# yanglei18/SGV3D

Measured on AMD Instinct MI355X. Metric: camera frames/sec at 864x1536->BEV, higher is better.
Workload: dtype f32

## Files before the change

include/sgv3d_hip.h:

```cpp
#ifndef SGV3D_HIP_H
#define SGV3D_HIP_H

#include <stddef.h>
#include <stdint.h>

#ifdef __cplusplus
extern "C" {
#endif

#define SGV3D_OK 0
#define SGV3D_EINVAL (-1)
#define SGV3D_ELAUNCH (-2)
#define SGV3D_ENOSPACE (-3)

const char *sgv3d_last_error(void);
int sgv3d_abi_version(void);


int sgv3d_voxel_pooling_forward(int batch_size, int num_points, int num_channels,
                                int num_voxel_x, int num_voxel_y, int num_voxel_z,
                                const int32_t *geom_xyz, const float *input_features,
                                float *output_features, int32_t *pos_memo, void *stream);
int sgv3d_voxel_pooling_forward_fresh(int batch_size, int num_points, int num_channels,
                                      int num_voxel_x, int num_voxel_y, int num_voxel_z,
// ... 193 lines not shown

int sgv3d_dense(int batch, int k, int n, const float *x, const float *w, const float *scale,
                const float *bias, int act, float *y, void *stream);
int sgv3d_dense_gated(int batch, int k, int n, const float *x, const float *w, const float *scale,
                      const float *bias, int act, float *y, const int32_t *run, void *stream);

int sgv3d_broadcast_channels(int batch, int pixels, int channels, int y_ld, int y_coff,
                             const float *v, float *y, void *stream);

int sgv3d_scale_channels(int batch, int pixels, int channels, const float *x, const float *gate,
                         float *y, void *stream);

int sgv3d_copy_channels(int batch, int pixels, int channels, int x_ld, int x_coff, const float *x,
                        float *y, void *stream);

int sgv3d_upsample_bilinear2x(int batch, int h, int w, int channels, const float *x, float *y, void *stream);

int sgv3d_add_mul_sigmoid(long long n, const float *a, const float *b, const float *c, float *y, void *stream);

int sgv3d_bsm_compose(int batch, int pixels, int num_depth, int context_channels, int semantic_channels,
                      int ld, const float *semantic_logits, int semantic_ld, float background_threshold,
                      float *height_context, void *stream);

int sgv3d_deform_conv3x3_forward(int batch, int h, int w, int channels, int groups, int out_per_group, const float *x,
                                 const float *offset, int off_ld, const float *const *w_packed, int k_pad, int cout_pad,
                                 float *y, int y_ld, int y_coff, void *stream);

size_t sgv3d_deform_conv3x3_bf16_weight_bytes(int channels, int groups, int out_per_group);
int sgv3d_deform_conv3x3_bf16_pack_weight(const float *weight, int channels, int groups, int out_per_group, void *w_packed,
                                          void *stream);
int sgv3d_deform_conv3x3_forward_bf16(int batch, int h, int w, int channels, int groups, int out_per_group, const void *x,
                                      int x_is_bf16, const float *offset, int off_ld, const void *w_packed, void *y,
                                      int y_is_bf16, int y_ld, int y_coff, void *stream);

int sgv3d_deform_im2col3x3(int batch, int h, int w, int channels, int groups, const float *x,
                           const float *offset, int off_ld, float *col, void *stream);

int sgv3d_head_final_conv(int batch, int h, int w, int num_branches, int hidden_ch, int total_out,
                          const float *hidden, const float *weight, const float *bias,
                          const int32_t *branch_of_out, float *out, void *stream);

size_t sgv3d_centerhead_branches_workspace_bytes(int batch, int h, int w, int total_out);
int sgv3d_centerhead_branches_forward(int batch, int h, int w, int cin, int x_ld, int x_coff, const float *x,
                                      int num_branches, const float *w1_wino, const float *scale1,
                                      const float *bias1, int total_out, const float *w2, const float *bias2,
                                      const int32_t *out_begin, float *out, void *workspace,
                                      size_t workspace_bytes, void *stream);

size_t sgv3d_centerhead_f4_weight_floats(int num_branches);
int sgv3d_centerhead_f4_pack_weight(const float *w1, int num_branches, float *u_packed, void *stream);
int sgv3d_centerhead_branches_forward_f4(int batch, int h, int w, int cin, int x_ld, int x_coff, const float *x,
                                         int num_branches, const float *u_packed, const float *scale1,
                                         const float *bias1, int total_out, const float *w2, const float *bias2,
                                         const int32_t *out_begin, float *out, void *workspace,
                                         size_t workspace_bytes, void *stream);

size_t sgv3d_conv3x3_f4res_weight_floats(int cout, int cin);
int sgv3d_conv3x3_f4res_pack_weight(const float *w, int cout, int cin_real, int cin, float *u_packed, void *stream);
int sgv3d_conv3x3_f4res_forward(const sgv3d_conv_desc *d, const float *x, const float *u_packed, const float *scale,
                                const float *bias, const float *residual, float *y, void *stream);

size_t sgv3d_centerhead_bf16_weight_bytes(int num_branches);
int sgv3d_centerhead_bf16_pack_weight(const float *w1, int num_branches, int cin, void *w1_packed, void *stream);
size_t sgv3d_centerhead_bf16_weight2_bytes(int num_branches);
int sgv3d_centerhead_bf16_pack_weight2(const float *w2, const int32_t *out_begin, int num_branches, void *w2_packed,
                                       void *stream);
// ... 451 lines not shown
```

sgv3d_amd/_lib.py:

```python
import ctypes
import os

_HERE = os.path.dirname(os.path.abspath(__file__))
LIB_PATH = os.path.join(_HERE, "csrc", "libsgv3d_hip.so")

c_int, c_void_p, c_size_t, c_ll = ctypes.c_int, ctypes.c_void_p, ctypes.c_size_t, ctypes.c_longlong


class ConvDesc(ctypes.Structure):
    _fields_ = [(n, c_int) for n in (
        "batch", "in_h", "in_w", "cin", "out_h", "out_w", "cout", "kh", "kw", "stride", "pad", "dil",
        "x_ld", "x_coff", "y_ld", "y_coff", "res_ld", "relu", "mode", "deconv_ks", "k_pad", "cout_pad",
        "tile", "x_nchw", "k_order", "split_k")]


class VitAttnDesc(ctypes.Structure):
    _fields_ = [(n, c_int) for n in ("batch", "height", "width", "heads", "head_dim", "win_h", "win_w")]


CONV_NORMAL, CONV_DECONV, CONV_NCHW_OUT, CONV_GROUP_PLANES = 0, 1, 2, 3
TILE_AUTO, TILE_128x128, TILE_128x64, TILE_64x128, TILE_64x64 = 0, 1, 2, 3, 4

_PROTOS = {
    "sgv3d_last_error": (ctypes.c_char_p, []),
# ... 69 lines not shown
    "sgv3d_conv_dw_bf16_forward_splitk": (c_int, [ctypes.POINTER(ConvDesc)] + [c_void_p] * 7 + [c_size_t, c_void_p]),
    "sgv3d_conv_dw_bf16_pair_forward": (c_int, [ctypes.POINTER(ConvDesc)] + [c_void_p] * 4 + [c_int] + [c_void_p] * 4 + [c_int, c_void_p, c_int, c_int, c_int, c_void_p]),
    "sgv3d_conv_winograd_weight_floats": (c_size_t, [c_int, c_int]),
    "sgv3d_conv_winograd_pack_weight": (c_int, [c_void_p, c_int, c_int, c_int, c_void_p, c_void_p]),
    "sgv3d_conv2d_winograd_forward": (c_int, [ctypes.POINTER(ConvDesc)] + [c_void_p] * 8 + [c_size_t, c_void_p]),
    "sgv3d_conv_winograd4_pack_weight": (c_int, [c_void_p, c_int, c_int, c_int, c_int, c_void_p, c_void_p]),
    "sgv3d_conv_winograd4_pack_weight_x3": (c_int, [c_void_p, c_int, c_int, c_int, c_int, c_void_p, c_void_p]),
    "sgv3d_conv_pack_weight_x3": (c_int, [c_void_p, c_int, c_int, c_int, c_int, c_int, c_int, c_void_p, c_void_p]),
    "sgv3d_conv2d_x3_forward": (c_int, [c_void_p] * 8 + [c_size_t, c_void_p]),
    "sgv3d_conv2d_x3_shortcut_forward": (c_int, [c_void_p] * 12),
    "sgv3d_stem_pool_x3_forward": (c_int, [c_int] * 3 + [c_void_p, c_void_p, c_size_t] + [c_void_p] * 3 + [c_int, c_int, c_void_p]),
    "sgv3d_conv2d_winograd4_workspace_bytes": (c_size_t, [ctypes.POINTER(ConvDesc)]),
    "sgv3d_conv2d_winograd4_forward": (c_int, [ctypes.POINTER(ConvDesc)] + [c_void_p] * 7 + [c_size_t, c_void_p]),
    "sgv3d_maxpool3x3s2": (c_int, [c_int] * 4 + [c_void_p] * 3),
    "sgv3d_maxpool3x3s2_bf16": (c_int, [c_int] * 4 + [c_void_p] * 3),
    "sgv3d_nchw_to_nhwc": (c_int, [c_int] * 5 + [c_void_p] * 3),
    "sgv3d_nhwc_to_nchw": (c_int, [c_int] * 6 + [c_void_p] * 3),
    "sgv3d_global_avgpool_workspace_bytes": (c_size_t, [c_int] * 2),
    "sgv3d_global_avgpool": (c_int, [c_int] * 4 + [c_void_p] * 3 + [c_size_t, c_void_p]),
    "sgv3d_dense": (c_int, [c_int] * 3 + [c_void_p] * 4 + [c_int, c_void_p, c_void_p]),
    "sgv3d_broadcast_channels": (c_int, [c_int] * 5 + [c_void_p] * 3),
    "sgv3d_scale_channels": (c_int, [c_int] * 3 + [c_void_p] * 4),
    "sgv3d_copy_channels": (c_int, [c_int] * 5 + [c_void_p] * 3),
    "sgv3d_upsample_bilinear2x": (c_int, [c_int] * 4 + [c_void_p] * 3),
    "sgv3d_add_mul_sigmoid": (c_int, [c_ll] + [c_void_p] * 5),
    "sgv3d_bsm_compose": (c_int, [c_int] * 6 + [c_void_p, c_int, ctypes.c_float, c_void_p, c_void_p]),
    "sgv3d_deform_im2col3x3": (c_int, [c_int] * 5 + [c_void_p, c_void_p, c_int, c_void_p, c_void_p]),
    "sgv3d_deform_conv3x3_forward": (c_int, [c_int] * 6 + [c_void_p, c_void_p, c_int, c_void_p, c_int, c_int, c_void_p, c_int, c_int,
                                                          c_void_p]),
    "sgv3d_deform_conv3x3_bf16_weight_bytes": (c_size_t, [c_int] * 3),
    "sgv3d_deform_conv3x3_bf16_pack_weight": (c_int, [c_void_p, c_int, c_int, c_int, c_void_p, c_void_p]),
    "sgv3d_deform_conv3x3_forward_bf16": (c_int, [c_int] * 6 + [c_void_p, c_int, c_void_p, c_int, c_void_p, c_void_p, c_int, c_int, c_int,
                                                               c_void_p]),
    "sgv3d_head_final_conv": (c_int, [c_int] * 6 + [c_void_p] * 6),
    "sgv3d_centerpoint_decode_workspace_bytes": (c_size_t, [c_int] * 3),
    "sgv3d_centerpoint_decode": (c_int, [c_int] * 5 + [c_void_p] * 6 + [c_ll] + [ctypes.c_float] * 6 +
                                 [ctypes.POINTER(ctypes.c_float), c_int, ctypes.c_float, c_int, c_void_p, c_size_t] +
                                 [c_void_p] * 6),
    "sgv3d_centerpoint_decode_tasks_workspace_bytes": (c_size_t, [c_int] * 4),
    "sgv3d_centerpoint_decode_tasks": (c_int, [c_int, c_int, ctypes.POINTER(ctypes.c_int32), c_int, c_int, c_int] +
                                       [ctypes.POINTER(c_void_p)] * 6 + [c_ll] + [ctypes.c_float] * 6 +
                                       [ctypes.POINTER(ctypes.c_float), c_int, ctypes.POINTER(ctypes.c_float), c_int, c_void_p,
                                        c_size_t] + [c_void_p] * 6),
    "sgv3d_centerpoint_merge_tasks": (c_int, [c_int] * 3 + [c_void_p] * 4 + [ctypes.POINTER(ctypes.c_int32)] + [c_void_p] * 5),
    "sgv3d_rotated_bev_iou_host": (c_int, [c_int] + [ctypes.POINTER(ctypes.c_float)] * 3),
    "sgv3d_rotate_nms_workspace_bytes": (c_size_t, [c_int] * 3),
    "sgv3d_rotate_nms": (c_int, [c_int] * 3 + [c_void_p] * 3 + [ctypes.c_float, ctypes.POINTER(ctypes.c_float), c_int, c_int,
                                                                ctypes.POINTER(ctypes.c_float), c_void_p, c_size_t, c_void_p, c_void_p]),
    "sgv3d_centerpoint_decode_tasks_rotate_workspace_bytes": (c_size_t, [c_int] * 4),
    "sgv3d_centerpoint_decode_tasks_rotate": (c_int, [c_int, c_int, ctypes.POINTER(ctypes.c_int32), c_int, c_int, c_int] +
                                              [ctypes.POINTER(c_void_p)] * 6 + [c_ll] + [ctypes.c_float] * 6 +
                                              [ctypes.POINTER(ctypes.c_float), c_int, ctypes.c_float, ctypes.POINTER(ctypes.c_float),
                                               c_int, c_int, ctypes.POINTER(ctypes.c_float), c_void_p, c_size_t] + [c_void_p] * 6),
    "sgv3d_centerhead_targets": (c_int, [c_int, c_int, c_void_p, c_void_p, c_int, ctypes.POINTER(ctypes.c_int32)] +
                                 [c_int] * 3 + [ctypes.c_float] * 5 + [ctypes.c_double, c_int, c_int] + [c_void_p] * 5),
    "sgv3d_conv2d_backward_weight_workspace_bytes": (c_size_t, [ctypes.POINTER(ConvDesc), c_int]),
    "sgv3d_conv2d_backward_weight": (c_int, [ctypes.POINTER(ConvDesc)] + [c_void_p] * 3 + [c_int, c_void_p, c_size_t, c_void_p]),
    "sgv3d_conv2d_backward_weight_bf16_workspace_bytes": (c_size_t, [ctypes.POINTER(ConvDesc), c_int]),
    "sgv3d_conv2d_backward_weight_bf16": (c_int, [ctypes.POINTER(ConvDesc)] + [c_void_p] * 3 + [c_int, c_void_p, c_size_t, c_void_p]),
    "sgv3d_conv2d_backward_weight_bf16_batched_workspace_bytes": (c_size_t, [ctypes.POINTER(ConvDesc), c_int, c_int]),
    "sgv3d_conv2d_backward_weight_bf16_batched": (c_int, [ctypes.POINTER(ConvDesc), c_void_p, ctypes.POINTER(c_void_p), ctypes.POINTER(c_void_p), c_int, c_int, c_void_p, c_size_t, c_void_p]),
    "sgv3d_conv2d_backward_weight_bf16_alltaps_workspace_bytes": (c_size_t, [ctypes.POINTER(ConvDesc), c_int, c_int]),
    "sgv3d_conv2d_backward_weight_bf16_alltaps": (c_int, [ctypes.POINTER(ConvDesc)] + [c_void_p] * 3 + [c_int, c_void_p, c_size_t, c_void_p]),
    "sgv3d_conv2d_backward_weight_bf16_tensors_workspace_bytes": (c_size_t, [ctypes.POINTER(ConvDesc), c_int]),
    "sgv3d_conv2d_backward_weight_bf16_tensors": (c_int, [ctypes.POINTER(ConvDesc)] + [c_void_p] * 3 + [c_int, c_void_p, c_size_t, c_void_p]),
    "sgv3d_conv2d_backward_weight_bf16_alltaps_tensors_workspace_bytes": (c_size_t, [ctypes.POINTER(ConvDesc), c_int]),
# ... 139 lines not shown
```

sgv3d_amd/csrc/dcn_fused_bf16.hip:

```cpp
#include "conv_common.hpp"

using namespace sgv3d;

namespace {

typedef float f32x4 __attribute__((ext_vector_type(4)));
typedef __bf16 bf16x8 __attribute__((ext_vector_type(8)));
typedef __bf16 bf16x4 __attribute__((ext_vector_type(4)));
typedef unsigned u32x4 __attribute__((ext_vector_type(4)));

constexpr int BK = 32;
constexpr int BM = 64;
constexpr int BN = 128;
constexpr int kThreads = 256;
constexpr int kMaxGroups = 8;
constexpr int kFragB = 64 * 16;
constexpr unsigned kOutside = 0x80000000u;

struct DcnBfArgs {
    const void *x;
    const float *off;
    const void *w;
    void *y;
    int H, W, C, cpg, opg, groups;
    int M;
    int off_ld, y_ld, y_coff;
    int nkt;
    int nchunk;
    int tiles_m;
    unsigned x_bytes, w_bytes;
};

__global__ __launch_bounds__(64) void dcn_bf16_pack_kernel(const float *__restrict__ w, int cpg, int opg, int nkt, int nblk,
                                                           __bf16 *__restrict__ out) {
    const int id = blockIdx.x;
    const int kt = id % nkt, gnb = id / nkt;
    const int nb = gnb % nblk, g = gnb / nblk;
    const int kpt = cpg / BK;
    const int tap = kt / kpt, cb = kt - tap * kpt;
    const int l = threadIdx.x;
    const int co = nb * 16 + (l & 15);
    __bf16 *dst = out + ((size_t)id * 64 + l) * 8;
#pragma unroll
    for (int j = 0; j < 8; ++j) {
        const int ci = cb * BK + 8 * (l >> 4) + j;
        dst[j] = co < opg ? (__bf16)w[((size_t)(g * opg + co) * cpg + ci) * 9 + tap] : (__bf16)0.f;
    }
}

__device__ __forceinline__ float as_f32(unsigned u) { return __builtin_bit_cast(float, u); }
// ... 42 lines not shown
        pw = (int)((unsigned)mm - t2 * a.W);
        const unsigned b = t2 / (unsigned)a.H;
        ph = (int)(t2 - b * a.H);
        pbase = (unsigned)(((size_t)b * a.H * a.W * a.C + (size_t)grp * a.cpg + c * 8) * ESZ);
    }
    char *const st_ptr = smem + r * (BK * 2) + ((c ^ ((r >> 2) & 3)) * 16);

    const int wave = tid >> 6, lane = tid & 63;
    const int l16 = lane & 15, lq = lane >> 4;
    const int rd_off = l16 * (BK * 2) + ((lq ^ ((l16 >> 2) & 3)) * 16);
    const int col0 = chunk * BN + 32 * wave;
    const bool live0 = col0 < a.opg, live1 = col0 + 16 < a.opg;
    const int nblk = 8 * a.nchunk;
    const int nb0 = grp * nblk + chunk * 8 + 2 * wave;
    const unsigned w_off0 = (unsigned)((size_t)nb0 * a.nkt * kFragB + lane * 16);
    const unsigned w_off1 = w_off0 + (unsigned)(a.nkt * kFragB);

    f32x4 acc[2][4];
#pragma unroll
    for (int nb = 0; nb < 2; ++nb)
#pragma unroll
        for (int mb = 0; mb < 4; ++mb) acc[nb][mb] = f32x4{0.f, 0.f, 0.f, 0.f};

    unsigned co[4];
    float cw[4];
    u32x4 rx[4][NLD];
    bf16x8 wc[2], wn[2];
    const int kpt = a.cpg / BK;
    int ld_kt = 0, ld_tap = 0, ld_c = 0;

    __syncthreads();

    auto tap_params = [&]() {
        const int ky = ld_tap / 3, kx = ld_tap - ky * 3;
        const float oy = off_s[r][2 * ld_tap], ox = off_s[r][2 * ld_tap + 1];
        const float hf = (float)(ph - 1 + ky) + oy;
        const float wf = (float)(pw - 1 + kx) + ox;
        const bool in = pok && hf > -1.f && wf > -1.f && hf < (float)a.H && wf < (float)a.W;
        const int hl = (int)floorf(hf), wl = (int)floorf(wf);
        const int hh = hl + 1, wh = wl + 1;
        const float lh = hf - (float)hl, lw = wf - (float)wl;
        const float uh = 1.f - lh, uw = 1.f - lw;
        const bool k1 = in && hl >= 0 && wl >= 0, k2 = in && hl >= 0 && wh <= a.W - 1;
        const bool k3 = in && hh <= a.H - 1 && wl >= 0, k4 = in && hh <= a.H - 1 && wh <= a.W - 1;
        cw[0] = k1 ? uh * uw : 0.f; cw[1] = k2 ? uh * lw : 0.f;
        cw[2] = k3 ? lh * uw : 0.f; cw[3] = k4 ? lh * lw : 0.f;
        const unsigned cb = (unsigned)a.C * (unsigned)ESZ;
        co[0] = k1 ? pbase + (unsigned)(hl * a.W + wl) * cb : kOutside;
        co[1] = k2 ? pbase + (unsigned)(hl * a.W + wh) * cb : kOutside;
        co[2] = k3 ? pbase + (unsigned)(hh * a.W + wl) * cb : kOutside;
        co[3] = k4 ? pbase + (unsigned)(hh * a.W + wh) * cb : kOutside;
    };
    auto load = [&]() {
        if (ld_c == 0) tap_params();
#pragma unroll
        for (int k = 0; k < 4; ++k)
#pragma unroll
            for (int i = 0; i < NLD; ++i)
                rx[k][i] = __builtin_bit_cast(u32x4, __builtin_amdgcn_raw_buffer_load_b128(x_rsrc, co[k] + 16 * i, ld_c * (BK * ESZ), 0));
        wn[0] = __builtin_bit_cast(bf16x8, __builtin_amdgcn_raw_buffer_load_b128(w_rsrc, w_off0, ld_kt * kFragB, 0));
        wn[1] = __builtin_bit_cast(bf16x8, __builtin_amdgcn_raw_buffer_load_b128(w_rsrc, w_off1, ld_kt * kFragB, 0));
        ++ld_kt;
        if (++ld_c == kpt) { ld_c = 0; ++ld_tap; }
    };
    auto combine_store = [&](int buf) {
        bf16x8 v;
#pragma unroll
        for (int e = 0; e < 8; ++e) {
            float v1, v2, v3, v4;
            if constexpr (XBF) {
                const int d = e >> 1;
                v1 = (e & 1) ? bf16_hi(rx[0][0][d]) : bf16_lo(rx[0][0][d]);
                v2 = (e & 1) ? bf16_hi(rx[1][0][d]) : bf16_lo(rx[1][0][d]);
                v3 = (e & 1) ? bf16_hi(rx[2][0][d]) : bf16_lo(rx[2][0][d]);
                v4 = (e & 1) ? bf16_hi(rx[3][0][d]) : bf16_lo(rx[3][0][d]);
            } else {
                v1 = as_f32(rx[0][e >> 2][e & 3]);
                v2 = as_f32(rx[1][e >> 2][e & 3]);
                v3 = as_f32(rx[2][e >> 2][e & 3]);
                v4 = as_f32(rx[3][e >> 2][e & 3]);
            }
            float s = cw[1] * v2;
            s = __builtin_fmaf(cw[0], v1, s);
            s = __builtin_fmaf(cw[2], v3, s);
            s = __builtin_fmaf(cw[3], v4, s);
            v[e] = (__bf16)s;
        }
        *reinterpret_cast<bf16x8 *>(st_ptr + buf * kBufB) = v;
    };

    load();
    combine_store(0);
    wc[0] = wn[0]; wc[1] = wn[1];
    __syncthreads();
    int buf = 0;
    for (int kt = 0; kt < a.nkt; ++kt) {
        const bool have_next = kt + 1 < a.nkt;
        if (have_next) load();
        bf16x8 fx[4];
#pragma unroll
        for (int mb = 0; mb < 4; ++mb) fx[mb] = *reinterpret_cast<const bf16x8 *>(smem + buf * kBufB + mb * 16 * (BK * 2) + rd_off);
        if (live0) {
#pragma unroll
            for (int mb = 0; mb < 4; ++mb) acc[0][mb] = __builtin_amdgcn_mfma_f32_16x16x32_bf16(wc[0], fx[mb], acc[0][mb], 0, 0, 0);
        }
        if (live1) {
#pragma unroll
            for (int mb = 0; mb < 4; ++mb) acc[1][mb] = __builtin_amdgcn_mfma_f32_16x16x32_bf16(wc[1], fx[mb], acc[1][mb], 0, 0, 0);
        }
        if (have_next) {
            combine_store(buf ^ 1);
            wc[0] = wn[0]; wc[1] = wn[1];
        }
        __syncthreads();
        buf ^= 1;
    }

#pragma unroll
    for (int nb = 0; nb < 2; ++nb) {
// ... 91 lines not shown
```

sgv3d_amd/hip_ops.py:

```python
import ctypes
from collections import namedtuple
from functools import partialmethod

import torch

from . import _lib, conv_tiles, pack_cache
from ._lib import ConvDesc, CONV_NORMAL, CONV_DECONV, CONV_NCHW_OUT, CONV_GROUP_PLANES
from .conv_tiles import (TILE_WINO, TILE_WINO_RES, TILE_PATCH, TILE_WINO_HALF, TILE_WINO4, TILE_WINO4_WIDE, TILE_WINO4_NARROW,
                         TILE_WINO4_OCC, TILE_WINO4_G48, TILE_F4RES)


def _st(t):
    return _lib.stream_handle(t.device)


PROFILE = None
AUTOTUNE = not __import__("os").environ.get("SGV3D_NO_AUTOTUNE")
DETERMINISTIC = __import__("os").environ.get("SGV3D_DETERMINISTIC", "0") not in ("", "0")


def deterministic():
    return DETERMINISTIC or torch.are_deterministic_algorithms_enabled()
PROFILE_DETAIL = False
import os as _os
# ... 847 lines not shown
    need = top + len(thunks) - 1
    while len(pool) < need:
        pool.append(distinct_stream(dev, pool))
    mine = pool[top:need]
    _BRANCH_TOP[key] = need
    cur = torch.cuda.current_stream(dev)
    results = [None] * len(thunks)
    try:
        for st, (i, t) in zip(mine, list(enumerate(thunks))[1:]):
            st.wait_stream(cur)
            with torch.cuda.stream(st):
                results[i] = t()
        results[0] = thunks[0]()
    finally:
        for st in mine:
            cur.wait_stream(st)
        _BRANCH_TOP[key] = top
    return results


_GRAPH_SPLIT_HOOK = None


def graph_split_point(tag):
    if _GRAPH_SPLIT_HOOK is not None:
        _GRAPH_SPLIT_HOOK(tag)


def switch_state():
    g = globals()
    return tuple(g.get(k) for k in ("AUTOTUNE", "SPLIT_K", "WINOGRAD", "FUSED_HEAD", "HEAD_PATH", "MFMA_BF16", "BF16_ACTIVATIONS",
                                    "MFMA_F32X3", "MFIRST", "WINO4", "WINO_HALF", "PATCH_BF16", "DW_BF16", "DW_DEEP", "DW_NARROW",
                                    "DW_SPLIT_K", "DW_DEEP_MAX_WGS", "PAIR_BF16", "TUNE_STREAMS", "PARALLEL_BRANCHES", "F4RES", "OCC5", "WINO4_G48", "DCN_FUSED", "WINO4_X3", "PW_X3",
                                    "DCN_FUSED_BF16", "DCN_FUSED_TRAIN", "TRAIN_BF16_STORAGE", "SHORTCUT_X3", "DECONV_X3", "VIT_BF16", "STEM_FUSED"))


def conv_pair_eligible(a, b, x, residual=None):
    return (MFMA_BF16 and not MFMA_F32X3 and DW_BF16 and PAIR_BF16 and x.dtype == torch.bfloat16 and not a.transposed and not b.transposed
            and a.cout == 256 and a.cin % 32 == 0 and int(x.shape[-1]) % 8 == 0 and b.cin == 256 and b.kh == 1 and b.kw == 1
            and b.stride == 1 and b.pad == 0 and b.cout % 256 == 0 and (residual is None or residual.dtype == torch.bfloat16))


def conv_pair_bf16(a, b, x, residual=None, out=None):
    B, H, W, x_ld = (int(v) for v in x.shape)
    oh, ow = a.out_hw(H, W)
    if out is None:
        out = torch.empty(B, oh, ow, b.cout, dtype=torch.bfloat16, device=x.device)
    d = ConvDesc()
    d.batch, d.in_h, d.in_w, d.cin = B, H, W, a.cin
    d.out_h, d.out_w, d.cout = oh, ow, a.cout
    d.kh, d.kw, d.stride, d.pad, d.dil = a.kh, a.kw, a.stride, a.pad, a.dil
    d.x_ld, d.x_coff, d.y_ld, d.y_coff = x_ld, 0, a.cout, 0
    d.relu, d.mode, d.split_k = (1 if a.relu else 0), CONV_NORMAL, 1
    flops = 2.0 * B * oh * ow * (a.cout_real * a.cin_real * a.kh * a.kw + b.cout_real * b.cin_real)
    name = "conv_dw_bf16_pair"
    if PROFILE_DETAIL:
        name += f"|{B}x{H}x{W}x{a.cin}->{a.cout} k{a.kh} s{a.stride} d{a.dil} ->{b.cout} k1"
    with torch.cuda.device(x.device), prof(name, flops):
        rc = _lib.load().sgv3d_conv_dw_bf16_pair_forward(
            ctypes.byref(d), x.data_ptr(), a._dw_weights().data_ptr(), _lib.ptr(a.scale), _lib.ptr(a.shift), b.cout,
            b._dw_weights().data_ptr(), _lib.ptr(b.scale), _lib.ptr(b.shift), _lib.ptr(residual),
            int(residual.shape[-1]) if residual is not None else 0, out.data_ptr(), int(out.shape[-1]), 0, 1 if b.relu else 0, _st(x))
    _lib.check(rc, "sgv3d_conv_dw_bf16_pair_forward")
    return out


def conv_pair_choice(a, b, x, residual=None):
# ... 526 lines not shown

def deform_conv3x3_bf16_covers(channels, groups, out_channels):
    C, g, cout = int(channels), int(groups), int(out_channels)
    return 0 < g <= 8 and C % g == 0 and (C // g) % 32 == 0 and cout % g == 0 and (cout // g) % 4 == 0


def deform_conv3x3_bf16_eligible(x, groups, out_channels):
    if not (DCN_FUSED and DCN_FUSED_BF16 and MFMA_BF16 and not MFMA_F32X3) or x.dim() != 4 or x.dtype not in (torch.bfloat16, torch.float32):
        return False
    return deform_conv3x3_bf16_covers(x.shape[-1], groups, out_channels)


def deform_conv3x3_bf16(x, offset, packed, out=None, y_coff=0, out_dtype=None):
    B, H, W, C = (int(v) for v in x.shape)
    g, opg = packed.groups, packed.opg
    assert C == packed.channels and x.dtype in (torch.bfloat16, torch.float32)
    assert x.is_contiguous() and offset.is_contiguous() and offset.dtype == torch.float32 and int(offset.shape[-1]) >= 18
    assert tuple(offset.shape[:3]) == (B, H, W)
    if out is None:
        out = torch.empty(B, H, W, g * opg, dtype=out_dtype or x.dtype, device=x.device)
    assert out.is_contiguous() and out.dtype in (torch.bfloat16, torch.float32) and tuple(out.shape[:3]) == (B, H, W)
    assert out_dtype is None or out.dtype == out_dtype
    flops = 2.0 * B * H * W * g * opg * 9 * (C // g)
    nbytes = (float(B * H * W) * (C * x.element_size() + 18 * 4 + g * opg * out.element_size()) + 2.0 * g * opg * 9 * (C // g))
    with torch.cuda.device(x.device), prof("conv_dcn_fused_bf16", flops, nbytes):
        rc = _lib.load().sgv3d_deform_conv3x3_forward_bf16(B, H, W, C, g, opg, x.data_ptr(), int(x.dtype == torch.bfloat16),
                                                          offset.data_ptr(), int(offset.shape[-1]), packed.w.data_ptr(),
                                                          out.data_ptr(), int(out.dtype == torch.bfloat16), int(out.shape[-1]),
                                                          int(y_coff), _st(x))
    _lib.check(rc, "sgv3d_deform_conv3x3_forward_bf16")
    return out


def deform_im2col3x3(x, offset, groups, out=None):
    B, H, W, C = (int(s) for s in x.shape)
    if out is None:
        out = torch.empty(B, H, W, 9 * C, dtype=x.dtype, device=x.device)
    assert offset.dtype == torch.float32 and out.dtype == x.dtype
    lib = _lib.load()
    fn = lib.sgv3d_deform_im2col3x3_bf16 if x.dtype == torch.bfloat16 else lib.sgv3d_deform_im2col3x3
    with torch.cuda.device(x.device), prof("deform_im2col3x3"):
        rc = fn(B, H, W, C, int(groups), x.data_ptr(), offset.data_ptr(), int(offset.shape[-1]), out.data_ptr(), _st(x))
    _lib.check(rc, "sgv3d_deform_im2col3x3")
    return out


HEAD_FINAL_MAX_OUT = 4


def head_branch_of_out(widths, device=None):
    widths = [int(c) for c in widths]
    if any(c < 0 or c > HEAD_FINAL_MAX_OUT for c in widths) or sum(widths) == 0:
        raise ValueError(f"head_final_conv: a branch has 0..{HEAD_FINAL_MAX_OUT} outputs and the head at least one, got {widths}")
    return torch.tensor([i for i, c in enumerate(widths) for _ in range(c)], dtype=torch.int32, device=device)


def head_final_conv(hidden, weight, bias, branch_of_out, num_branches, hidden_ch, out=None):
    nb, B, H, W, hc = (int(s) for s in hidden.shape)
    assert nb == num_branches and hc == hidden_ch and _dense_layout(hidden)
    total = int(weight.shape[0])
    assert _dense_layout(weight) and tuple(weight.shape) == (total, 3, 3, hc)
    assert _dense_layout(bias) and bias.numel() == total
    assert _dense_layout(branch_of_out, torch.int32) and branch_of_out.numel() == total
    if out is None:
        out = torch.empty(B, total, H, W, dtype=torch.float32, device=hidden.device)
    assert _dense_layout(out) and out.numel() == B * total * H * W
# ... 105 lines not shown
```

sgv3d_amd/layers/backbones/lss_fpn.py:

```python
import ctypes

import numpy as np
import torch
from torch import nn

from ... import _lib, hip_ops
from ...hip_ops import PackedConv, fold_bn
from ...calibration import CalibrationCache
from ...ops.voxel_pooling import VoxelPlan
from ..blocks import BasicBlock, HipModule, build_backbone, build_neck, conv_bn

import os as _os

CACHE_CAMERA_GATES = _os.environ.get("SGV3D_CACHE_CAMERA_GATES", "1") != "0"
GATED_CALIBRATION = _os.environ.get("SGV3D_GATED_CALIBRATION", "1") != "0"
FOLD_ASPP_POOL = _os.environ.get("SGV3D_FOLD_ASPP_POOL", "1") != "0"
FUSE_LIFT_SPLAT = _os.environ.get("SGV3D_FUSE_LIFT_SPLAT", "1") != "0"

__all__ = ['LSSFPN']


class _ASPPModule(HipModule):

    def __init__(self, inplanes, planes, kernel_size, padding, dilation, BatchNorm):
# ... 88 lines not shown
    def __init__(self, channels, act_layer=nn.ReLU, gate_layer=nn.Sigmoid):
        super().__init__()
        self.conv_reduce = nn.Conv2d(channels, channels, 1, bias=True)
        self.act1 = act_layer()
        self.conv_expand = nn.Conv2d(channels, channels, 1, bias=True)
        self.gate = gate_layer()


class DCN(HipModule):

    def __init__(self, in_channels, out_channels, kernel_size=3, padding=1, groups=1, deform_groups=1,
                 stride=1, dilation=1, im2col_step=32, **unused):
        super().__init__()
        assert kernel_size == 3 and padding == 1 and stride == 1 and dilation == 1 and deform_groups == 1
        assert in_channels % groups == 0 and out_channels % groups == 0
        self.in_channels, self.out_channels, self.groups = in_channels, out_channels, groups
        self.weight = nn.Parameter(torch.empty(out_channels, in_channels // groups, 3, 3))
        nn.init.kaiming_uniform_(self.weight, nonlinearity='relu')
        self.conv_offset = nn.Conv2d(in_channels, deform_groups * 2 * 9, kernel_size=3, stride=1, padding=1, bias=True)
        nn.init.zeros_(self.conv_offset.weight)
        nn.init.zeros_(self.conv_offset.bias)

    def hip_compile(self, device):
        g = self.groups
        opg, cpg = self.out_channels // g, self.in_channels // g
        convs = []
        for gi in range(g):
            wg = self.weight.detach()[gi * opg:(gi + 1) * opg]
            wg = wg.permute(0, 2, 3, 1).reshape(opg, 9 * cpg, 1, 1).contiguous()
            convs.append(PackedConv(wg, device=device))
        dcn_bf16 = None
        if hip_ops.deform_conv3x3_bf16_covers(self.in_channels, g, self.out_channels):
            dcn_bf16 = hip_ops.PackedDeformBf16(self.weight, g, device=device)
        return dict(offset=conv_bn(self.conv_offset, None, False, device), convs=convs, opg=opg, cpg=cpg, dcn_bf16=dcn_bf16)

    def hip_forward(self, x):
        s = self.hip_state(x.device)
        B, H, W, C = x.shape
        offset = s['offset'](x)
        if hip_ops.deform_conv3x3_eligible(x, s['convs']):
            return hip_ops.deform_conv3x3(x, offset, s['convs'])
        if s['dcn_bf16'] is not None and hip_ops.deform_conv3x3_bf16_eligible(x, self.groups, self.out_channels):
            return hip_ops.deform_conv3x3_bf16(x, offset, s['dcn_bf16'])
        col = hip_ops.deform_im2col3x3(x, offset, self.groups)
        out = torch.empty(B, H, W, self.out_channels, dtype=x.dtype, device=x.device)
        for gi, conv in enumerate(s['convs']):
            conv(col, out, x_coff=gi * 9 * s['cpg'], y_coff=gi * s['opg'])
        return out


class HeightNet(HipModule):

    def __init__(self, in_channels, mid_channels, context_channels, height_channels):
        super().__init__()
        self.reduce_conv = nn.Sequential(
            nn.Conv2d(in_channels, mid_channels, kernel_size=3, stride=1, padding=1),
            nn.BatchNorm2d(mid_channels),
            nn.ReLU(inplace=True),
        )
        self.context_conv = nn.Conv2d(mid_channels, context_channels, kernel_size=1, stride=1, padding=0)
        self.bn = nn.BatchNorm1d(27)
        self.height_mlp = Mlp(27, mid_channels, mid_channels)
        self.height_se = SELayer(mid_channels)
        self.context_mlp = Mlp(27, mid_channels, mid_channels)
        self.context_se = SELayer(mid_channels)
        self.height_conv = nn.Sequential(
            BasicBlock(mid_channels, mid_channels),
            BasicBlock(mid_channels, mid_channels),
            BasicBlock(mid_channels, mid_channels),
            ASPP(mid_channels, mid_channels),
            DCN(in_channels=mid_channels, out_channels=mid_channels, kernel_size=3, padding=1, groups=4,
                im2col_step=128),
# ... 305 lines not shown
```

Baseline: 292.5.

## Add fused deformable conv kernel using split-bf16 x3 MFMA for f32 accuracy

Adds a fused deformable 3x3 convolution kernel that samples bilinear inputs and splits both activations and weights into three bf16 parts (hi/mid/lo). It runs six bf16 MFMA products per step to emulate f32 precision on matrix cores. The intent is to replace the existing f32 fused DCN path with faster bf16 matrix instructions while keeping close-to-f32 accuracy. The new path is picked per shape by autotuning against the f32 kernel and falls back when it is not faster. It costs extra weight storage and sixfold MFMA work, and the shared sampling code is moved into a common header.

```diff
diff --git a/include/sgv3d_hip.h b/include/sgv3d_hip.h
--- a/include/sgv3d_hip.h
+++ b/include/sgv3d_hip.h
@@ -249,6 +249,13 @@
 int sgv3d_deform_conv3x3_forward_bf16(int batch, int h, int w, int channels, int groups, int out_per_group, const void *x,
                                       int x_is_bf16, const float *offset, int off_ld, const void *w_packed, void *y,
                                       int y_is_bf16, int y_ld, int y_coff, void *stream);
+
+size_t sgv3d_deform_conv3x3_x3_weight_bytes(int channels, int groups, int out_per_group);
+int sgv3d_deform_conv3x3_x3_pack_weight(const float *weight, int channels, int groups, int out_per_group, void *w_packed,
+                                        void *stream);
+int sgv3d_deform_conv3x3_forward_x3(int batch, int h, int w, int channels, int groups, int out_per_group, const float *x,
+                                    const float *offset, int off_ld, const void *w_packed, float *y, int y_ld, int y_coff,
+                                    int tile_pixels, void *stream);
 
 int sgv3d_deform_im2col3x3(int batch, int h, int w, int channels, int groups, const float *x,
                            const float *offset, int off_ld, float *col, void *stream);
diff --git a/sgv3d_amd/_lib.py b/sgv3d_amd/_lib.py
--- a/sgv3d_amd/_lib.py
+++ b/sgv3d_amd/_lib.py
@@ -125,6 +125,9 @@
     "sgv3d_deform_conv3x3_bf16_pack_weight": (c_int, [c_void_p, c_int, c_int, c_int, c_void_p, c_void_p]),
     "sgv3d_deform_conv3x3_forward_bf16": (c_int, [c_int] * 6 + [c_void_p, c_int, c_void_p, c_int, c_void_p, c_void_p, c_int, c_int, c_int,
                                                                c_void_p]),
+    "sgv3d_deform_conv3x3_x3_weight_bytes": (c_size_t, [c_int] * 3),
+    "sgv3d_deform_conv3x3_x3_pack_weight": (c_int, [c_void_p, c_int, c_int, c_int, c_void_p, c_void_p]),
+    "sgv3d_deform_conv3x3_forward_x3": (c_int, [c_int] * 6 + [c_void_p, c_void_p, c_int, c_void_p, c_void_p, c_int, c_int, c_int, c_void_p]),
     "sgv3d_head_final_conv": (c_int, [c_int] * 6 + [c_void_p] * 6),
     "sgv3d_centerpoint_decode_workspace_bytes": (c_size_t, [c_int] * 3),
     "sgv3d_centerpoint_decode": (c_int, [c_int] * 5 + [c_void_p] * 6 + [c_ll] + [ctypes.c_float] * 6 +
diff --git a/sgv3d_amd/csrc/dcn_fused_bf16.hip b/sgv3d_amd/csrc/dcn_fused_bf16.hip
--- a/sgv3d_amd/csrc/dcn_fused_bf16.hip
+++ b/sgv3d_amd/csrc/dcn_fused_bf16.hip
@@ -1,4 +1,5 @@
 #include "conv_common.hpp"
+#include "dcn_sample.hpp"
 
 using namespace sgv3d;
 
@@ -15,7 +16,6 @@
 constexpr int kThreads = 256;
 constexpr int kMaxGroups = 8;
 constexpr int kFragB = 64 * 16;
-constexpr unsigned kOutside = 0x80000000u;
 
 struct DcnBfArgs {
     const void *x;
@@ -124,24 +124,7 @@
     __syncthreads();
 
     auto tap_params = [&]() {
-        const int ky = ld_tap / 3, kx = ld_tap - ky * 3;
-        const float oy = off_s[r][2 * ld_tap], ox = off_s[r][2 * ld_tap + 1];
-        const float hf = (float)(ph - 1 + ky) + oy;
-        const float wf = (float)(pw - 1 + kx) + ox;
-        const bool in = pok && hf > -1.f && wf > -1.f && hf < (float)a.H && wf < (float)a.W;
-        const int hl = (int)floorf(hf), wl = (int)floorf(wf);
-        const int hh = hl + 1, wh = wl + 1;
-        const float lh = hf - (float)hl, lw = wf - (float)wl;
-        const float uh = 1.f - lh, uw = 1.f - lw;
-        const bool k1 = in && hl >= 0 && wl >= 0, k2 = in && hl >= 0 && wh <= a.W - 1;
-        const bool k3 = in && hh <= a.H - 1 && wl >= 0, k4 = in && hh <= a.H - 1 && wh <= a.W - 1;
-        cw[0] = k1 ? uh * uw : 0.f; cw[1] = k2 ? uh * lw : 0.f;
-        cw[2] = k3 ? lh * uw : 0.f; cw[3] = k4 ? lh * lw : 0.f;
-        const unsigned cb = (unsigned)a.C * (unsigned)ESZ;
-        co[0] = k1 ? pbase + (unsigned)(hl * a.W + wl) * cb : kOutside;
-        co[1] = k2 ? pbase + (unsigned)(hl * a.W + wh) * cb : kOutside;
-        co[2] = k3 ? pbase + (unsigned)(hh * a.W + wl) * cb : kOutside;
-        co[3] = k4 ? pbase + (unsigned)(hh * a.W + wh) * cb : kOutside;
+        dcn_tap_params(ld_tap, off_s[r][2 * ld_tap], off_s[r][2 * ld_tap + 1], ph, pw, pok, a.H, a.W, pbase, (unsigned)a.C * (unsigned)ESZ, co, cw);
     };
     auto load = [&]() {
         if (ld_c == 0) tap_params();
@@ -172,11 +155,7 @@
                 v3 = as_f32(rx[2][e >> 2][e & 3]);
                 v4 = as_f32(rx[3][e >> 2][e & 3]);
             }
-            float s = cw[1] * v2;
-            s = __builtin_fmaf(cw[0], v1, s);
-            s = __builtin_fmaf(cw[2], v3, s);
-            s = __builtin_fmaf(cw[3], v4, s);
-            v[e] = (__bf16)s;
+            v[e] = (__bf16)dcn_bilinear(cw, v1, v2, v3, v4);
         }
         *reinterpret_cast<bf16x8 *>(st_ptr + buf * kBufB) = v;
     };
diff --git a/sgv3d_amd/csrc/dcn_fused_x3.hip b/sgv3d_amd/csrc/dcn_fused_x3.hip
--- /dev/null
+++ b/sgv3d_amd/csrc/dcn_fused_x3.hip
@@ -0,0 +1,279 @@
+#include "conv_common.hpp"
+#include "dcn_sample.hpp"
+
+using namespace sgv3d;
+
+namespace {
+
+typedef float f32x4 __attribute__((ext_vector_type(4)));
+typedef __bf16 bf16x8 __attribute__((ext_vector_type(8)));
+typedef unsigned u32x4 __attribute__((ext_vector_type(4)));
+
+constexpr int BK = 32;
+constexpr int BN = 128;
+constexpr int kThreads = 256;
+constexpr int kMaxGroups = 8;
+constexpr int kFragB = 64 * 16;
+constexpr int kStepB = 3 * kFragB;
+
+struct DcnX3Args {
+    const float *x;
+    const float *off;
+    const void *w;
+    float *y;
+    int H, W, C, cpg, opg, groups;
+    int M;
+    int off_ld, y_ld, y_coff;
+    int nkt;
+    int nchunk;
+    int tiles_m;
+    unsigned x_bytes, w_bytes;
+};
+
+__global__ __launch_bounds__(64) void dcn_x3_pack_kernel(const float *__restrict__ w, int cpg, int opg, int nkt, int nblk,
+                                                         __bf16 *__restrict__ out) {
+    const int id = blockIdx.x;
+    const int kt = id % nkt, gnb = id / nkt;
+    const int nb = gnb % nblk, g = gnb / nblk;
+    const int kpt = cpg / BK;
+    const int tap = kt / kpt, cb = kt - tap * kpt;
+    const int l = threadIdx.x;
+    const int co = nb * 16 + (l & 15);
+    __bf16 *dst = out + ((size_t)id * 3 * 64 + l) * 8;
+#pragma unroll
+    for (int j = 0; j < 8; ++j) {
+        const int ci = cb * BK + 8 * (l >> 4) + j;
+        const float v = co < opg ? w[((size_t)(g * opg + co) * cpg + ci) * 9 + tap] : 0.f;
+        const __bf16 hi = (__bf16)v;
+        const float r1 = v - (float)hi;
+        const __bf16 mid = (__bf16)r1;
+        const float r2 = r1 - (float)mid;
+        dst[j] = hi;
+        dst[512 + j] = mid;
+        dst[1024 + j] = (__bf16)r2;
+    }
+}
+
+__device__ __forceinline__ float as_f32(unsigned u) { return __builtin_bit_cast(float, u); }
+
+template <int BM>
+__global__ __launch_bounds__(kThreads, 2) void dcn3x3_fused_x3_kernel(const DcnX3Args a) {
+    static_assert(BM == 64 || BM == 32, "pixels per workgroup");
+    constexpr int CPT = BM / 8;
+    constexpr int TPR = BK / CPT;
+    constexpr int NLD = CPT / 4;
+    constexpr int MB = BM / 16;
+    constexpr int kPlaneB = BM * BK * 2;
+    constexpr int kBufB = 3 * kPlaneB;
+    typedef float fvec __attribute__((ext_vector_type(CPT)));
+    typedef __bf16 bvec __attribute__((ext_vector_type(CPT)));
+    __shared__ __attribute__((aligned(16))) char smem[2 * kBufB];
+    __shared__ float off_s[BM][18];
+
+    const int per_m = a.groups * a.nchunk;
+    const int ntiles = a.tiles_m * per_m;
+    const int bid = blockIdx.x;
+    const int xcd = bid & 7, idx = bid >> 3;
+    const int q8 = ntiles >> 3, r8 = ntiles & 7;
+    const int logical = (xcd < r8 ? xcd * (q8 + 1) : r8 * (q8 + 1) + (xcd - r8) * q8) + idx;
+    const int tgc = (int)((unsigned)logical / (unsigned)a.tiles_m);
+    const int tm = logical - tgc * a.tiles_m;
+    const int grp = tgc / a.nchunk;
+    const int chunk = tgc - grp * a.nchunk;
+    const int m0 = tm * BM;
+
+    const int tid = threadIdx.x;
+    const int c = tid % TPR, r = tid / TPR;
+
+    for (int i = tid; i < BM * 18; i += kThreads) {
+        const int rr = i / 18, cc = i - rr * 18;
+        const int m = m0 + rr;
+        off_s[rr][cc] = m < a.M ? a.off[(size_t)m * a.off_ld + cc] : 0.f;
+    }
+
+    const __amdgpu_buffer_rsrc_t x_rsrc = __builtin_amdgcn_make_buffer_rsrc((void *)a.x, 0, (int)a.x_bytes, 0x00020000);
+    const __amdgpu_buffer_rsrc_t w_rsrc = __builtin_amdgcn_make_buffer_rsrc((void *)a.w, 0, (int)a.w_bytes, 0x00020000);
+
+    const int m_row = m0 + r;
+    const bool pok = m_row < a.M;
+    int ph, pw;
+    unsigned pbase;
+    {
+        const int mm = pok ? m_row : 0;
+        const unsigned t2 = (unsigned)mm / (unsigned)a.W;
+        pw = (int)((unsigned)mm - t2 * a.W);
+        const unsigned b = t2 / (unsigned)a.H;
+        ph = (int)(t2 - b * a.H);
+        pbase = (unsigned)(((size_t)b * a.H * a.W * a.C + (size_t)grp * a.cpg + c * CPT) * 4);
+    }
+    const int piece = c * CPT * 2;
+    char *const st_ptr = smem + r * (BK * 2) + ((((piece >> 4) ^ ((r >> 2) & 3)) << 4) | (piece & 15));
+
+    const int wave = tid >> 6, lane = tid & 63;
+    const int l16 = lane & 15, lq = lane >> 4;
+    const int rd_off = l16 * (BK * 2) + ((lq ^ ((l16 >> 2) & 3)) * 16);
+    const int col0 = chunk * BN + 32 * wave;
+    const bool live0 = col0 < a.opg, live1 = col0 + 16 < a.opg;
+    const int nblk = 8 * a.nchunk;
+    const int nb0 = grp * nblk + chunk * 8 + 2 * wave;
+    const unsigned w_off0 = (unsigned)((size_t)nb0 * a.nkt * kStepB + lane * 16);
+    const unsigned w_off1 = w_off0 + (unsigned)(a.nkt * kStepB);
+
+    f32x4 acc[2][MB];
+#pragma unroll
+    for (int nb = 0; nb < 2; ++nb)
+#pragma unroll
+        for (int mb = 0; mb < MB; ++mb) acc[nb][mb] = f32x4{0.f, 0.f, 0.f, 0.f};
+
+    unsigned co[4];
+    float cw[4];
+    u32x4 rx[4][NLD];
+    bf16x8 wa[2][3], wb[2][3];
+    const int kpt = a.cpg / BK;
+    int ld_kt = 0, ld_tap = 0, ld_c = 0;
+
+    __syncthreads();
+
+    auto load = [&](bf16x8 (&wn)[2][3]) {
+        if (ld_c == 0)
+            dcn_tap_params(ld_tap, off_s[r][2 * ld_tap], off_s[r][2 * ld_tap + 1], ph, pw, pok, a.H, a.W, pbase, (unsigned)a.C * 4u, co, cw);
+#pragma unroll
+        for (int k = 0; k < 4; ++k)
+#pragma unroll
+            for (int i = 0; i < NLD; ++i)
+                rx[k][i] = __builtin_bit_cast(u32x4, __builtin_amdgcn_raw_buffer_load_b128(x_rsrc, co[k] + 16 * i, ld_c * (BK * 4), 0));
+#pragma unroll
+        for (int s = 0; s < 3; ++s) {
+            wn[0][s] = __builtin_bit_cast(bf16x8, __builtin_amdgcn_raw_buffer_load_b128(w_rsrc, w_off0 + s * kFragB, ld_kt * kStepB, 0));
+            wn[1][s] = __builtin_bit_cast(bf16x8, __builtin_amdgcn_raw_buffer_load_b128(w_rsrc, w_off1 + s * kFragB, ld_kt * kStepB, 0));
+        }
+        ++ld_kt;
+        if (++ld_c == kpt) { ld_c = 0; ++ld_tap; }
+    };
+    auto combine_store = [&](int buf) {
+        fvec s;
+#pragma unroll
+        for (int e = 0; e < CPT; ++e)
+            s[e] = dcn_bilinear(cw, as_f32(rx[0][e >> 2][e & 3]), as_f32(rx[1][e >> 2][e & 3]), as_f32(rx[2][e >> 2][e & 3]),
+                                as_f32(rx[3][e >> 2][e & 3]));
+        const bvec hi = __builtin_convertvector(s, bvec);
+        const fvec r1 = s - __builtin_convertvector(hi, fvec);
+        const bvec mid = __builtin_convertvector(r1, bvec);
+        const fvec r2 = r1 - __builtin_convertvector(mid, fvec);
+        const bvec lo = __builtin_convertvector(r2, bvec);
+        char *d = st_ptr + buf * kBufB;
+        *reinterpret_cast<bvec *>(d) = hi;
+        *reinterpret_cast<bvec *>(d + kPlaneB) = mid;
+        *reinterpret_cast<bvec *>(d + 2 * kPlaneB) = lo;
+    };
+    auto products = [&](const bf16x8 (&w)[3], const bf16x8 (&fx)[MB][3], f32x4 (&ac)[MB]) {
+        constexpr int wp[6] = {2, 0, 1, 1, 0, 0}, xp[6] = {0, 2, 1, 0, 1, 0};
+#pragma unroll
+        for (int p = 0; p < 6; ++p)
+#pragma unroll
+            for (int mb = 0; mb < MB; ++mb) ac[mb] = __builtin_amdgcn_mfma_f32_16x16x32_bf16(w[wp[p]], fx[mb][xp[p]], ac[mb], 0, 0, 0);
+    };
+    auto phase = [&](int buf, bool have_next, const bf16x8 (&wc)[2][3], bf16x8 (&wn)[2][3]) {
+        if (have_next) load(wn);
+        bf16x8 fx[MB][3];
+#pragma unroll
+        for (int mb = 0; mb < MB; ++mb)
+#pragma unroll
+            for (int s = 0; s < 3; ++s)
+                fx[mb][s] = *reinterpret_cast<const bf16x8 *>(smem + buf * kBufB + s * kPlaneB + mb * 16 * (BK * 2) + rd_off);
+        if (live0) products(wc[0], fx, acc[0]);
+        if (have_next) combine_store(buf ^ 1);
+        if (live1) products(wc[1], fx, acc[1]);
+        __syncthreads();
+    };
+
+    load(wa);
+    combine_store(0);
+    __syncthreads();
+    for (int kt = 0; kt < a.nkt; kt += 2) {
+        phase(0, kt + 1 < a.nkt, wa, wb);
+        if (kt + 1 >= a.nkt) break;
+        phase(1, kt + 2 < a.nkt, wb, wa);
+    }
+
+#pragma unroll
+    for (int nb = 0; nb < 2; ++nb) {
+        const int col = col0 + 16 * nb + 4 * lq;
+        if (col >= a.opg) continue;
+        const size_t ybase = (size_t)(m0 + l16) * a.y_ld + a.y_coff + grp * a.opg + col;
+#pragma unroll
+        for (int mb = 0; mb < MB; ++mb) {
+            if (m0 + 16 * mb + l16 >= a.M) continue;
+            *reinterpret_cast<f32x4 *>(a.y + ybase + (size_t)mb * 16 * a.y_ld) = acc[nb][mb];
+        }
+    }
+}
+
+bool dcn_x3_geometry(int channels, int groups, int out_per_group, int *nkt, int *nblk, long long *bytes) {
+    if (channels <= 0 || groups <= 0 || groups > kMaxGroups || channels % groups || out_per_group <= 0) return false;
+    const int cpg = channels / groups;
+    if (cpg % BK || out_per_group % 4) return false;
+    *nkt = 9 * (cpg / BK);
+    *nblk = 8 * cdiv(out_per_group, BN);
+    *bytes = (long long)groups * *nblk * *nkt * kStepB;
+    return *bytes < 0x7fffff00LL;
+}
+
+}
+
+extern "C" size_t sgv3d_deform_conv3x3_x3_weight_bytes(int channels, int groups, int out_per_group) {
+    int nkt, nblk;
+    long long bytes;
+    return dcn_x3_geometry(channels, groups, out_per_group, &nkt, &nblk, &bytes) ? (size_t)bytes : 0;
+}
+
+extern "C" int sgv3d_deform_conv3x3_x3_pack_weight(const float *weight, int channels, int groups, int out_per_group, void *w_packed,
+                                                   void *stream) {
+    int nkt = 0, nblk = 0;
+    long long bytes = 0;
+    SGV3D_REQUIRE(dcn_x3_geometry(channels, groups, out_per_group, &nkt, &nblk, &bytes),
+                  "deform_conv3x3_x3_pack_weight: groups <= 8, channels %% groups == 0, channels per group %% 32, outputs per group %% 4 "
+                  "(channels=%d groups=%d opg=%d)", channels, groups, out_per_group);
+    SGV3D_REQUIRE(weight && w_packed, "deform_conv3x3_x3_pack_weight: null pointer");
+    hipLaunchKernelGGL(dcn_x3_pack_kernel, dim3(groups * nblk * nkt), dim3(64), 0, as_stream(stream), weight, channels / groups,
+                       out_per_group, nkt, nblk, static_cast<__bf16 *>(w_packed));
+    return check_launch("dcn_x3_pack_kernel");
+}
+
+extern "C" int sgv3d_deform_conv3x3_forward_x3(int batch, int h, int w, int channels, int groups, int out_per_group, const float *x,
+                                               const float *offset, int off_ld, const void *w_packed, float *y, int y_ld, int y_coff,
+                                               int tile_pixels, void *stream) {
+    SGV3D_REQUIRE(batch > 0 && h > 0 && w > 0 && channels > 0 && groups > 0 && groups <= kMaxGroups && channels % groups == 0 &&
+                      out_per_group > 0 && off_ld >= 18,
+                  "deform_conv3x3_forward_x3: bad shape");
+    SGV3D_REQUIRE(tile_pixels == 64 || tile_pixels == 32, "deform_conv3x3_forward_x3: 64 or 32 pixels per workgroup (tile_pixels=%d)",
+                  tile_pixels);
+    int nkt = 0, nblk = 0;
+    long long w_bytes = 0;
+    SGV3D_REQUIRE(dcn_x3_geometry(channels, groups, out_per_group, &nkt, &nblk, &w_bytes) && y_coff >= 0 && (y_ld & 3) == 0 &&
+                      (y_coff & 3) == 0 && y_ld >= y_coff + groups * out_per_group,
+                  "deform_conv3x3_forward_x3: channels per group %% 32, outputs per group %% 4, output stride / offset %% 4 "
+                  "(cpg=%d opg=%d y_ld=%d y_coff=%d)", channels / groups, out_per_group, y_ld, y_coff);
+    SGV3D_REQUIRE(x && offset && w_packed && y, "deform_conv3x3_forward_x3: null pointer");
+    const long long M = (long long)batch * h * w;
+    const long long x_bytes = M * channels * 4;
+    SGV3D_REQUIRE(M < 0x7fffffffLL && x_bytes < 0x7fffff00LL && M * y_ld < 0x7fffffffLL,
+                  "deform_conv3x3_forward_x3: input map larger than 2 GiB (32-bit buffer offsets)");
+    SGV3D_REQUIRE(((reinterpret_cast<uintptr_t>(x) | reinterpret_cast<uintptr_t>(y) | reinterpret_cast<uintptr_t>(w_packed)) & 15) == 0,
+                  "deform_conv3x3_forward_x3: pointers must be 16-B aligned");
+    DcnX3Args a;
+    a.x = x; a.off = offset; a.w = w_packed; a.y = y;
+    a.H = h; a.W = w; a.C = channels; a.cpg = channels / groups; a.opg = out_per_group; a.groups = groups;
+    a.M = (int)M; a.off_ld = off_ld; a.y_ld = y_ld; a.y_coff = y_coff;
+    a.nkt = nkt; a.nchunk = nblk / 8;
+    a.tiles_m = cdiv(M, tile_pixels);
+    a.x_bytes = (unsigned)x_bytes;
+    a.w_bytes = (unsigned)w_bytes;
+    const long long grid = (long long)a.tiles_m * groups * a.nchunk;
+    SGV3D_REQUIRE(grid < 0x7fffffffLL, "deform_conv3x3_forward_x3: too many tiles");
+    const dim3 g((unsigned)grid), b(kThreads);
+    hipStream_t s = as_stream(stream);
+    if (tile_pixels == 64) hipLaunchKernelGGL((dcn3x3_fused_x3_kernel<64>), g, b, 0, s, a);
+    else hipLaunchKernelGGL((dcn3x3_fused_x3_kernel<32>), g, b, 0, s, a);
+    return check_launch("dcn3x3_fused_x3_kernel");
+}
diff --git a/sgv3d_amd/csrc/dcn_sample.hpp b/sgv3d_amd/csrc/dcn_sample.hpp
--- /dev/null
+++ b/sgv3d_amd/csrc/dcn_sample.hpp
@@ -0,0 +1,35 @@
+#pragma once
+
+namespace sgv3d {
+
+constexpr unsigned kDcnOutside = 0x80000000u;
+
+__device__ __forceinline__ void dcn_tap_params(int tap, float oy, float ox, int ph, int pw, bool pok, int H, int W, unsigned pbase,
+                                               unsigned cb, unsigned (&co)[4], float (&cw)[4]) {
+    const int ky = tap / 3, kx = tap - ky * 3;
+    const float hf = (float)(ph - 1 + ky) + oy;
+    const float wf = (float)(pw - 1 + kx) + ox;
+    const bool in = pok && hf > -1.f && wf > -1.f && hf < (float)H && wf < (float)W;
+    const int hl = (int)floorf(hf), wl = (int)floorf(wf);
+    const int hh = hl + 1, wh = wl + 1;
+    const float lh = hf - (float)hl, lw = wf - (float)wl;
+    const float uh = 1.f - lh, uw = 1.f - lw;
+    const bool k1 = in && hl >= 0 && wl >= 0, k2 = in && hl >= 0 && wh <= W - 1;
+    const bool k3 = in && hh <= H - 1 && wl >= 0, k4 = in && hh <= H - 1 && wh <= W - 1;
+    cw[0] = k1 ? uh * uw : 0.f; cw[1] = k2 ? uh * lw : 0.f;
+    cw[2] = k3 ? lh * uw : 0.f; cw[3] = k4 ? lh * lw : 0.f;
+    co[0] = k1 ? pbase + (unsigned)(hl * W + wl) * cb : kDcnOutside;
+    co[1] = k2 ? pbase + (unsigned)(hl * W + wh) * cb : kDcnOutside;
+    co[2] = k3 ? pbase + (unsigned)(hh * W + wl) * cb : kDcnOutside;
+    co[3] = k4 ? pbase + (unsigned)(hh * W + wh) * cb : kDcnOutside;
+}
+
+__device__ __forceinline__ float dcn_bilinear(const float (&cw)[4], float v1, float v2, float v3, float v4) {
+    float s = cw[1] * v2;
+    s = __builtin_fmaf(cw[0], v1, s);
+    s = __builtin_fmaf(cw[2], v3, s);
+    s = __builtin_fmaf(cw[3], v4, s);
+    return s;
+}
+
+}
diff --git a/sgv3d_amd/hip_ops.py b/sgv3d_amd/hip_ops.py
--- a/sgv3d_amd/hip_ops.py
+++ b/sgv3d_amd/hip_ops.py
@@ -903,7 +903,7 @@
     return tuple(g.get(k) for k in ("AUTOTUNE", "SPLIT_K", "WINOGRAD", "FUSED_HEAD", "HEAD_PATH", "MFMA_BF16", "BF16_ACTIVATIONS",
                                     "MFMA_F32X3", "MFIRST", "WINO4", "WINO_HALF", "PATCH_BF16", "DW_BF16", "DW_DEEP", "DW_NARROW",
                                     "DW_SPLIT_K", "DW_DEEP_MAX_WGS", "PAIR_BF16", "TUNE_STREAMS", "PARALLEL_BRANCHES", "F4RES", "OCC5", "WINO4_G48", "DCN_FUSED", "WINO4_X3", "PW_X3",
-                                    "DCN_FUSED_BF16", "DCN_FUSED_TRAIN", "TRAIN_BF16_STORAGE", "SHORTCUT_X3", "DECONV_X3", "VIT_BF16", "STEM_FUSED"))
+                                    "DCN_FUSED_BF16", "DCN_FUSED_TRAIN", "TRAIN_BF16_STORAGE", "SHORTCUT_X3", "DECONV_X3", "VIT_BF16", "STEM_FUSED", "DCN_X3"))
 
 
 def conv_pair_eligible(a, b, x, residual=None):
@@ -1496,6 +1496,96 @@
     return out
 
 
+DCN_X3 = _os.environ.get("SGV3D_DCN_X3", "1") != "0"
+DCN_X3_VARIANTS = (64, 32)
+
+
+class PackedDeformX3:
+
+    def __init__(self, weight, groups, device=None):
+        w = weight.detach()
+        device = device or w.device
+        w = w.to(device=device, dtype=torch.float32).contiguous()
+        cout, cpg, kh, kw = (int(v) for v in w.shape)
+        assert kh == 3 and kw == 3 and cout % int(groups) == 0
+        self.groups, self.channels, self.opg = int(groups), cpg * int(groups), cout // int(groups)
+        lib = _lib.load()
+        nbytes = int(lib.sgv3d_deform_conv3x3_x3_weight_bytes(self.channels, self.groups, self.opg))
+        if nbytes == 0:
+            raise _lib.SGV3DError(f"deform_conv3x3_x3: shape not covered (channels={self.channels} groups={self.groups} "
+                                  f"outputs per group={self.opg})")
+        self.w = torch.empty(nbytes // 2, dtype=torch.bfloat16, device=device)
+        with torch.cuda.device(device):
+            rc = lib.sgv3d_deform_conv3x3_x3_pack_weight(w.data_ptr(), self.channels, self.groups, self.opg, self.w.data_ptr(), _st(w))
+        _lib.check(rc, "sgv3d_deform_conv3x3_x3_pack_weight")
+        self._keep = w
+
+
+def deform_conv3x3_x3_weight_bytes(channels, groups, out_channels):
+    C, g, cout = int(channels), int(groups), int(out_channels)
+    return g * 8 * -(-(cout // g) // 128) * (9 * (C // g) // 32) * 3072
+
+
+def deform_conv3x3_x3_eligible(x, groups, out_channels):
+    if not (DCN_FUSED and DCN_X3 and PW_X3 and not MFMA_BF16 and not MFMA_F32X3) or x.dim() != 4 or x.dtype != torch.float32:
+        return False
+    return deform_conv3x3_bf16_covers(x.shape[-1], groups, out_channels)
+
+
+def deform_conv3x3_x3(x, offset, packed, out=None, y_coff=0, variant=None):
+    B, H, W, C = (int(v) for v in x.shape)
+    g, opg = packed.groups, packed.opg
+    variant = int(variant or DCN_X3_VARIANTS[0])
+    if variant not in DCN_X3_VARIANTS:
+        raise _lib.SGV3DError(f"deform_conv3x3_x3: unknown variant {variant}")
+    assert C == packed.channels and x.dtype == torch.float32
+    assert x.is_contiguous() and offset.is_contiguous() and offset.dtype == torch.float32 and int(offset.shape[-1]) >= 18
+    assert tuple(offset.shape[:3]) == (B, H, W)
+    if out is None:
+        out = torch.empty(B, H, W, g * opg, dtype=torch.float32, device=x.device)
+    assert out.is_contiguous() and out.dtype == torch.float32 and tuple(out.shape[:3]) == (B, H, W)
+    cpg = C // g
+    flops = 2.0 * B * H * W * g * opg * 9 * cpg
+    nbytes = 4.0 * (B * H * W * (C + 18 + g * opg) + g * opg * 9 * cpg)
+    extra = None
+    if PROFILE is not None:
+        mfma = 2.0 * -(-B * H * W // variant) * variant * g * -(-opg // 128) * 128 * 9 * cpg
+        extra = {"symbol": f"dcn3x3_fused_x3_kernel<{variant}>", "mfma_flops": mfma, "bf16_mfma_flops": 6 * mfma}
+    with torch.cuda.device(x.device), prof("conv_dcn_fused_x3", flops, nbytes, extra):
+        rc = _lib.load().sgv3d_deform_conv3x3_forward_x3(B, H, W, C, g, opg, x.data_ptr(), offset.data_ptr(), int(offset.shape[-1]),
+                                                        packed.w.data_ptr(), out.data_ptr(), int(out.shape[-1]), int(y_coff), variant,
+                                                        _st(x))
+    _lib.check(rc, "sgv3d_deform_conv3x3_forward_x3")
+    return out
+
+
+def dcn_x3_signature(x, groups, out_channels):
+    B, H, W, C = (int(v) for v in x.shape)
+    return f"pair|dcn|{int(out_channels)}x{C}g{int(groups)}|{B}x{H}x{W}|ts{TUNE_STREAMS}"
+
+
+def dcn_x3_choice(x, offset, convs, packed):
+    if packed is None or not deform_conv3x3_x3_eligible(x, packed.groups, packed.groups * packed.opg):
+        return None
+    rule = DCN_X3_VARIANTS[0]
+    sig = dcn_x3_signature(x, packed.groups, packed.groups * packed.opg)
+    hit = tune_lookup(sig, x.device)
+    if hit is not None:
+        on, v = (int(t) for t in hit)
+        if not on:
+            return None
+        return v if v in DCN_X3_VARIANTS else rule
+    if not tune_may_measure() or not deform_conv3x3_eligible(x, convs):
+        return rule
+    TUNE_STATS["measured"] += 1
+    out = torch.empty(tuple(x.shape[:3]) + (packed.groups * packed.opg,), dtype=torch.float32, device=x.device)
+    t32, best, t1 = tune_best_of(sig, x.device, lambda: deform_conv3x3(x, offset, convs, out=out),
+                                 [(v, lambda v=v: deform_conv3x3_x3(x, offset, packed, out=out, variant=v)) for v in DCN_X3_VARIANTS])
+    on = t1 < t32
+    tune_record(sig, [1, best] if on else [0, 0])
+    return best if on else None
+
+
 def deform_im2col3x3(x, offset, groups, out=None):
     B, H, W, C = (int(s) for s in x.shape)
     if out is None:
diff --git a/sgv3d_amd/layers/backbones/lss_fpn.py b/sgv3d_amd/layers/backbones/lss_fpn.py
--- a/sgv3d_amd/layers/backbones/lss_fpn.py
+++ b/sgv3d_amd/layers/backbones/lss_fpn.py
@@ -144,12 +144,19 @@
         dcn_bf16 = None
         if hip_ops.deform_conv3x3_bf16_covers(self.in_channels, g, self.out_channels):
             dcn_bf16 = hip_ops.PackedDeformBf16(self.weight, g, device=device)
-        return dict(offset=conv_bn(self.conv_offset, None, False, device), convs=convs, opg=opg, cpg=cpg, dcn_bf16=dcn_bf16)
+        dcn_x3 = None
+        if hip_ops.deform_conv3x3_bf16_covers(self.in_channels, g, self.out_channels):
+            dcn_x3 = hip_ops.PackedDeformX3(self.weight, g, device=device)
+        return dict(offset=conv_bn(self.conv_offset, None, False, device), convs=convs, opg=opg, cpg=cpg, dcn_bf16=dcn_bf16,
+                    dcn_x3=dcn_x3)
 
     def hip_forward(self, x):
         s = self.hip_state(x.device)
         B, H, W, C = x.shape
         offset = s['offset'](x)
+        x3 = hip_ops.dcn_x3_choice(x, offset, s['convs'], s['dcn_x3'])
+        if x3 is not None:
+            return hip_ops.deform_conv3x3_x3(x, offset, s['dcn_x3'], variant=x3)
         if hip_ops.deform_conv3x3_eligible(x, s['convs']):
             return hip_ops.deform_conv3x3(x, offset, s['convs'])
         if s['dcn_bf16'] is not None and hip_ops.deform_conv3x3_bf16_eligible(x, self.groups, self.out_channels):
```

New measurement: 292.7 (median of 2 runs). No clear change (+0.1%).
